# openpifpaf/openpifpaf

Measured on AMD Instinct MI355X. Metric: images/sec end-to-end (backbone+CifCaf decode), resnet50 641px, higher is better.
Workload: dtype f32; 1 GPU; BASELINE configs[1] scaled to a batch: resnet50 641x641, batch 32 per GPU, CIF/CAF fields [32,17,5,81,81]+[32,19,8,81,81]; backbone=resnet50, backbone_dtype=fp32, conv3x3=winograd F(2x2,3x3) f32 for the stride-1 ones, decode_dtype=f32 (+f64 where the reference uses double), global_batch=32, batch_per_gpu=32, parallelism=single GPU, force_complete_pose=False

## Files before the change

openpifpaf_amd/csrc/gemm_f32x3.hip:

```cpp
#include <cstdlib>
#include <type_traits>
#include "common.hpp"
#include "split_bf16.hpp"

namespace opa {

typedef __attribute__((ext_vector_type(8))) __bf16 bf16x8_t;
typedef __attribute__((ext_vector_type(16))) float f32x16_t;
typedef __attribute__((ext_vector_type(4))) float f32x4_t;
typedef __attribute__((ext_vector_type(4))) unsigned int u32x4_t;
typedef __attribute__((ext_vector_type(2))) unsigned int u32x2_t;
typedef __attribute__((ext_vector_type(2))) float f32x2_t;

#ifndef OPA_X3_BK
#define OPA_X3_BK 32
#endif
#ifndef OPA_X3_WGS
#define OPA_X3_WGS 2
#endif
#ifndef OPA_X3_DIAG
#define OPA_X3_DIAG 0
#endif
#ifndef OPA_X3_ONE_ACC
#define OPA_X3_ONE_ACC 0
#endif
#ifndef OPA_X3_SWIZZLE
#define OPA_X3_SWIZZLE 1
#endif
constexpr int kX3BM = 128, kX3BK = OPA_X3_BK, kX3Pitch = OPA_X3_SWIZZLE ? kX3BK : kX3BK + 8;
__device__ __forceinline__ int x3_lds(int row, int k) {
    if (OPA_X3_SWIZZLE && kX3BK == 32) return row * kX3Pitch + ((((k >> 3) ^ (row >> 2)) & 3) << 3) + (k & 7);
    return row * kX3Pitch + k;
}

struct X3Second {
    const float* A2 = nullptr;
    int K1 = 0;
    int ho_wo = 1, wo = 1, hi_wi = 1, wi = 1, stride = 1;
    int hi = 1, C = 0, batch = 1;
    int pix = 1, taps_x = 1, ntaps = 1, padded = 0;
    int dil = 1;
    int lda = 0, ldp = 0, n_real = 0, k_real = 0;
    int act = 0; float act_param = 0.0f;
};

constexpr int kUxAct = 3, kUxHardswish = 2, kUxResidual = 4, kUxActParam = 8;

template <int BN, bool PARTNER, bool RELU, int UX = 0>
__device__ __forceinline__ void x3_unit_epilogue(float* smem_f, const f32x16_t (&acc)[2][BN / 64], const f32x16_t (&low)[2][BN / 64],
                                                 const float* __restrict__ bias, const float* __restrict__ partner,
                                                 float* __restrict__ out, int M, int m0, int n0, int lane, int wave, int ldp, int n_real,
                                                 int act, float act_param) {
    constexpr int WN = BN / 2, NT = WN / 32;
    constexpr int PPR = WN / 2;
    constexpr int PPL = 32 * PPR / 64;
    constexpr int PPRE = PPL > 8 ? 8 : PPL;
    const int wm = wave >> 1, wn = wave & 1;
    float* patch = smem_f + wave * (32 * WN);
#pragma unroll
    for (int i = 0; i < 2; i++) {
        f32x2_t pv[PPRE];
        if (PARTNER) {
#pragma unroll
            for (int t = 0; t < PPRE; t++) {
                const int v = t * 64 + lane;
                const int row = v / PPR, col = n0 + wn * WN + (v % PPR) * 2;
                const int m = m0 + wm * 64 + i * 32 + row;
                pv[t] = (f32x2_t){0.f, 0.f};
                if (m < M && col < n_real) pv[t] = *reinterpret_cast<const f32x2_t*>(partner + (size_t)m * ldp + col);
            }
        }
#pragma unroll
        for (int j = 0; j < NT; j++) {
            const int col = j * 32 + (lane & 31);
            const float b = bias[n0 + wn * WN + col];
#pragma unroll
            for (int r = 0; r < 16; r++) {
                const int row = (r & 3) + 8 * (r >> 2) + 4 * (lane >> 5);
                patch[row * WN + col] = (OPA_X3_ONE_ACC ? acc[i][j][r] : acc[i][j][r] + low[i][j][r]) + b;
            }
        }
        __builtin_amdgcn_fence(__ATOMIC_ACQ_REL, "wavefront");
        __builtin_amdgcn_wave_barrier();
#pragma unroll
        for (int t = 0; t < PPL; t++) {
            const int v = t * 64 + lane;
            const int row = v / PPR, c2 = (v % PPR) * 2, col = n0 + wn * WN + c2;
            const int m = m0 + wm * 64 + i * 32 + row;
            if (m < M && col < n_real) {
                f32x2_t f = *reinterpret_cast<const f32x2_t*>(patch + row * WN + c2);
                if constexpr (PARTNER && (UX & kUxResidual) != 0) {
                    f32x2_t pp;
                    if (t < PPRE) pp = pv[t < PPRE ? t : 0];
                    else pp = *reinterpret_cast<const f32x2_t*>(partner + (size_t)m * ldp + col);
                    f[0] += pp[0]; f[1] += pp[1];
                }
                if (RELU) { f[0] = fmaxf(f[0], 0.0f); f[1] = fmaxf(f[1], 0.0f); }
                if constexpr ((UX & kUxAct) == kUxHardswish) { f[0] = hardswish_f32(f[0]); f[1] = hardswish_f32(f[1]); }
                if constexpr ((UX & kUxActParam) != 0) { f[0] = x3_act_param(f[0], act, act_param); f[1] = x3_act_param(f[1], act, act_param); }
                if (PARTNER && (UX & kUxResidual) == 0) {
                    f32x2_t pp;
                    if (t < PPRE) pp = pv[t < PPRE ? t : 0];
                    else pp = *reinterpret_cast<const f32x2_t*>(partner + (size_t)m * ldp + col);
                    *reinterpret_cast<f32x4_t*>(out + (size_t)m * (2 * (size_t)n_real) + 2 * col) = (f32x4_t){pp[0], f[0], pp[1], f[1]};
                } else {
                    *reinterpret_cast<f32x2_t*>(out + (size_t)m * n_real + col) = f;
                }
            }
        }
        __builtin_amdgcn_fence(__ATOMIC_ACQ_REL, "wavefront");
        __builtin_amdgcn_wave_barrier();
        asm volatile("" ::: "memory");
    }
}

template <int BN, bool RES, bool RELU, bool PRO, int TERMS, int SRC, bool UNIT = false, int UX = 0>
__global__ __launch_bounds__(256, OPA_X3_WGS) void gemm_f32x3_bias_act_kernel(
        const float* __restrict__ A, const unsigned short* __restrict__ W3, const float* __restrict__ bias,
        const float* __restrict__ res, float* __restrict__ out, int M, int N, int K, const float* __restrict__ a_bias,
        const X3Second sec) {
    constexpr int WN = BN / 2;
    constexpr int NT = WN / 32;
    constexpr int LDS_A = kX3BM * kX3Pitch, LDS_B = BN * kX3Pitch;
#ifndef OPA_X3_PAD_LDS
#define OPA_X3_PAD_LDS 0
#endif
    constexpr int STAGE_BYTES = 3 * (LDS_A + LDS_B) * 2 + OPA_X3_PAD_LDS;
    constexpr int EPI_BYTES = 4 * 32 * WN * 4;
    constexpr int SMEM_BYTES = STAGE_BYTES > EPI_BYTES ? STAGE_BYTES : EPI_BYTES;
    __shared__ __attribute__((aligned(16))) unsigned char smem[SMEM_BYTES + (RES && !UNIT ? BN * 4 : 0)];
    unsigned short* sA = reinterpret_cast<unsigned short*>(smem);
    unsigned short* sB = sA + 3 * LDS_A;

    const int tid = threadIdx.x, lane = tid & 63, wave = tid >> 6;
    const int wm = wave >> 1, wn = wave & 1;
    const int n_tiles = N / BN;
    const unsigned nwg = gridDim.x, xcd = blockIdx.x & 7u, in_xcd = blockIdx.x >> 3;
    const unsigned q = nwg >> 3, r8 = nwg & 7u;
    const unsigned logical = (xcd < r8 ? xcd * (q + 1) : r8 * (q + 1) + (xcd - r8) * q) + in_xcd;
    const int m0 = (int)(logical / n_tiles) * kX3BM;
    const int n0 = (int)(logical % n_tiles) * BN;

    constexpr int NL = OPA_X3_ONE_ACC ? 1 : 2;
    f32x16_t acc[2][NT], low_[NL][NT];
    f32x16_t (&low)[2][NT] = OPA_X3_ONE_ACC ? acc : reinterpret_cast<f32x16_t (&)[2][NT]>(low_);
#pragma unroll
    for (int i = 0; i < 2; i++)
#pragma unroll
        for (int j = 0; j < NT; j++)
#pragma unroll
            for (int r = 0; r < 16; r++) { acc[i][j][r] = 0.0f; if (!OPA_X3_ONE_ACC) low[i][j][r] = 0.0f; }

    constexpr int VA = kX3BK / 4;
    constexpr int RPP = 256 / VA;
    constexpr int NPA = kX3BM / RPP;
    constexpr int WQ = kX3BK / 8;
    const int s_row = tid / VA, s_col = (tid % VA) * 4;
    constexpr int WTOT = 3 * BN * WQ;
    constexpr int WV = (WTOT + 255) / 256;
    f32x4_t ra0[NPA], ra1[NPA];
    u32x4_t rb[WV];
    constexpr bool TWO = SRC == 1, TAPS = SRC == 2;
    const int rows_here = M - m0 < kX3BM ? M - m0 : kX3BM;
    const int KA = TWO ? sec.K1 : TAPS ? sec.C : UNIT ? sec.lda : K;
    const int shift = TAPS && !sec.padded ? sec.dil * (sec.wi + 1) * sec.pix : 0;
    const float* a1_base = TAPS ? A - (size_t)shift : A + (size_t)m0 * KA;
    const int a1_bytes = TAPS ? (int)(((size_t)sec.batch * sec.hi_wi * sec.pix + shift) * 4)
                       : UNIT ? (int)(((size_t)(rows_here - 1) * KA + sec.k_real) * 4) : (int)((size_t)rows_here * KA * 4);
    const __amdgpu_buffer_rsrc_t a_rsrc = __builtin_amdgcn_make_buffer_rsrc(const_cast<float*>(a1_base), 0, a1_bytes, 0x00020000);
    const int K2 = K - KA;
    auto in_row = [&](int m) -> long long {
        const int b = m / sec.ho_wo, r = m - b * sec.ho_wo, oy = r / sec.wo, ox = r - oy * sec.wo;
        return (long long)b * sec.hi_wi + (long long)oy * sec.stride * sec.wi + (long long)ox * sec.stride;
    };
    long long row0_2 = 0;
    const float* a2_base = nullptr;
    int a2_bytes = 0;
    unsigned pa2[NPA];
    if constexpr (TWO) {
        row0_2 = in_row(__builtin_amdgcn_readfirstlane(m0));
        const int m_end = m0 + rows_here - 1;
        a2_base = sec.A2 + (size_t)row0_2 * K2;
        a2_bytes = (int)((size_t)(in_row(__builtin_amdgcn_readfirstlane(m_end)) - row0_2 + 1) * K2 * 4);
    }
    const __amdgpu_buffer_rsrc_t w_rsrc = __builtin_amdgcn_make_buffer_rsrc(
        const_cast<unsigned short*>(W3 + (size_t)n0 * K), 0, (int)(((size_t)3 * N - n0) * K * 2), 0x00020000);
    unsigned pa[NPA], pb[WV];
    unsigned vmask[NPA];
    int sb_off[WV];
#pragma unroll
    for (int p = 0; p < NPA; p++) {
        int m = m0 + p * RPP + s_row;
        if (m > M - 1) m = M - 1;
        pa[p] = ((unsigned)(m - m0) * (unsigned)KA + (unsigned)s_col) * 4u;
        vmask[p] = 0u;
        if constexpr (TAPS) {
            const int b = m / sec.ho_wo, r = m - b * sec.ho_wo, oy = r / sec.wo, ox = r - oy * sec.wo;
            pa[p] = (unsigned)((long long)b * sec.hi_wi + (long long)oy * sec.stride * sec.wi + (long long)ox * sec.stride) * (unsigned)sec.pix * 4u
                    + (unsigned)s_col * 4u;
            if (sec.padded) vmask[p] = 0xffffffffu;
            else
                for (int t = 0; t < sec.ntaps; t++) {
                    const int iy = oy * sec.stride - sec.dil + sec.dil * (t / sec.taps_x), ix = ox * sec.stride - sec.dil + sec.dil * (t % sec.taps_x);
                    if (iy >= 0 && iy < sec.hi && ix >= 0 && ix < sec.wi) vmask[p] |= 1u << t;
                }
        }
        if constexpr (TWO) pa2[p] = ((unsigned)(in_row(m) - row0_2) * (unsigned)K2 + (unsigned)s_col) * 4u;
    }
#pragma unroll
    for (int t = 0; t < WV; t++) {
        const int v = t * 256 + tid < WTOT ? t * 256 + tid : WTOT - 1;
        const int plane = v / (BN * WQ), rem = v - plane * (BN * WQ), row = rem / WQ, c = (rem % WQ) * 8;
        pb[t] = (((unsigned)plane * (unsigned)N + (unsigned)row) * (unsigned)K + (unsigned)c) * 2u;
        sb_off[t] = plane * LDS_B + x3_lds(row, c);
    }
    auto fetch_a = [&](f32x4_t (&ra)[NPA], int k0) {
        if constexpr (TAPS) {
            const int t = k0 / KA, kc = k0 - t * KA;
            const int soff = (int)((((unsigned)(sec.dil * (t / sec.taps_x)) * (unsigned)sec.wi + (unsigned)(sec.dil * (t % sec.taps_x))) * (unsigned)sec.pix + (unsigned)kc) * 4u);
#pragma unroll
            for (int p = 0; p < NPA; p++)
                ra[p] = __builtin_bit_cast(f32x4_t, __builtin_amdgcn_raw_buffer_load_b128(a_rsrc, (vmask[p] >> t) & 1u ? pa[p] : 0xFFFFFFF0u, soff, 0));
        } else if constexpr (TWO) {
            const bool second = k0 >= KA;
            const __amdgpu_buffer_rsrc_t rs = __builtin_amdgcn_make_buffer_rsrc(
                const_cast<float*>(second ? a2_base : a1_base), 0, second ? a2_bytes : a1_bytes, 0x00020000);
            const int ks = (second ? k0 - KA : k0) * 4;
#pragma unroll
            for (int p = 0; p < NPA; p++)
                ra[p] = __builtin_bit_cast(f32x4_t, __builtin_amdgcn_raw_buffer_load_b128(rs, second ? pa2[p] : pa[p], ks, 0));
        } else if constexpr (UNIT) {
#pragma unroll
            for (int p = 0; p < NPA; p++) {
                const f32x2_t lo = __builtin_bit_cast(f32x2_t, __builtin_amdgcn_raw_buffer_load_b64(a_rsrc, pa[p], k0 * 4, 0));
                const f32x2_t hi = __builtin_bit_cast(f32x2_t, __builtin_amdgcn_raw_buffer_load_b64(a_rsrc, pa[p] + 8u, k0 * 4, 0));
                ra[p] = (f32x4_t){lo[0], lo[1], hi[0], hi[1]};
            }
        } else {
#pragma unroll
            for (int p = 0; p < NPA; p++) ra[p] = __builtin_bit_cast(f32x4_t, __builtin_amdgcn_raw_buffer_load_b128(a_rsrc, pa[p], k0 * 4, 0));
        }
        if (PRO) {
            const f32x4_t ab = *reinterpret_cast<const f32x4_t*>(a_bias + k0 + s_col);
#pragma unroll
            for (int p = 0; p < NPA; p++)
#pragma unroll
                for (int e = 0; e < 4; e++) ra[p][e] = fmaxf(ra[p][e] + ab[e], 0.0f);
        }
    };
    auto fetch_b = [&](int k0) {
#pragma unroll
        for (int t = 0; t < WV; t++) rb[t] = __builtin_bit_cast(u32x4_t, __builtin_amdgcn_raw_buffer_load_b128(w_rsrc, pb[t], k0 * 2, 0));
    };
    auto store = [&](const f32x4_t (&ra)[NPA], int kt) {
#pragma unroll
        for (int p = 0; p < NPA; p++) {
            u32x2_t p1, p2, p3;
            if (OPA_X3_DIAG == 1) { p1[0] = __float_as_uint(ra[p][0]); p1[1] = __float_as_uint(ra[p][2]); p2 = p1; p3 = p1; }
            else if constexpr (UNIT) {
                const bool in0 = kt + s_col < sec.k_real, in1 = kt + s_col + 2 < sec.k_real;
                const f32x4_t v = {in0 ? ra[p][0] : 0.0f, in0 ? ra[p][1] : 0.0f, in1 ? ra[p][2] : 0.0f, in1 ? ra[p][3] : 0.0f};
                split4(v, p1, p2, p3);
            }
            else split4(ra[p], p1, p2, p3);
            unsigned short* d = sA + x3_lds(p * RPP + s_row, s_col);
            *reinterpret_cast<u32x2_t*>(d) = p1;
            *reinterpret_cast<u32x2_t*>(d + LDS_A) = p2;
            *reinterpret_cast<u32x2_t*>(d + 2 * LDS_A) = p3;
        }
#pragma unroll
        for (int t = 0; t < WV; t++)
            if (WTOT % 256 == 0 || t * 256 + tid < WTOT) *reinterpret_cast<u32x4_t*>(sB + sb_off[t]) = rb[t];
    };
    constexpr int VEC_PER_ROW = WN / 4;
    constexpr int VPL = 32 * VEC_PER_ROW / 64;
    constexpr int VRA = 1;
    constexpr bool TAIL_RES = RES && !UNIT;
    f32x4_t rres[2][TAIL_RES ? VPL : 1];
    auto fetch_res = [&](int i, int t_begin, int t_end) {
        if constexpr (TAIL_RES) {
            const __amdgpu_buffer_rsrc_t r_rsrc = __builtin_amdgcn_make_buffer_rsrc(
                const_cast<float*>(res + (size_t)m0 * N + n0), 0, (int)(((size_t)(rows_here - 1) * N + BN) * 4), 0x00020000);
            const int lrow = wm * 64 + lane / VEC_PER_ROW;
            const unsigned off = ((unsigned)lrow * (unsigned)N + (unsigned)(wn * WN + (lane % VEC_PER_ROW) * 4)) * 4u;
#pragma unroll
            for (int t = t_begin; t < t_end; t++) {
                const int urow = i * 32 + t * (64 / VEC_PER_ROW);
                rres[i][t] = __builtin_bit_cast(f32x4_t, __builtin_amdgcn_raw_buffer_load_b128(
                    r_rsrc, lrow < rows_here - urow ? off : 0xFFFFFFF0u, urow * N * 4, 0));
            }
        }
    };
    int frag_a[kX3BK / 16], frag_b[kX3BK / 16];
    if constexpr (TAIL_RES) {
#pragma unroll
        for (int h = 0; h < kX3BK / 16; h++) {
            frag_a[h] = 2 * x3_lds(wm * 64 + (lane & 31), h * 16 + (lane >> 5) * 8);
            frag_b[h] = 2 * x3_lds(wn * WN + (lane & 31), h * 16 + (lane >> 5) * 8);
            asm volatile("" : "+v"(frag_a[h]), "+v"(frag_b[h]));
        }
    }
    auto step = [&](auto tail, int k0, f32x4_t (&cur)[NPA], f32x4_t (&nxt)[NPA]) {
        constexpr int TAIL = decltype(tail)::value;
        const bool more = TAIL == 1 || (TAIL == 0 && k0 + kX3BK < K);
        const int k_last = K - kX3BK;
        if constexpr (TAIL == 0) {
            fetch_b(k0 + kX3BK < k_last ? k0 + kX3BK : k_last);
            fetch_a(nxt, k0 + 2 * kX3BK < k_last ? k0 + 2 * kX3BK : k_last);
        } else if constexpr (TAIL == 1) {
            fetch_b(k_last);
            fetch_res(0, 0, VRA);
        } else {
            fetch_res(0, VRA, VPL);
        }
        __builtin_amdgcn_sched_barrier(0);
#pragma unroll
        for (int kk = 0; kk < kX3BK; kk += 16) {
            bf16x8_t fa[3][2], fb[3][NT];
            const int kh = OPA_X3_DIAG == 4 ? 0 : kk / 16;
            const int kof = kh * 16 + (lane >> 5) * 8;
#pragma unroll
            for (int pl = 0; pl < 3; pl++) {
#pragma unroll
                for (int i = 0; i < 2; i++)
                    fa[pl][i] = *reinterpret_cast<const bf16x8_t*>(TAIL_RES ? reinterpret_cast<const unsigned short*>(smem + frag_a[kh]) + (pl * LDS_A + i * 32 * kX3Pitch)
                                                                       : sA + pl * LDS_A + x3_lds(wm * 64 + i * 32 + (lane & 31), kof));
#pragma unroll
                for (int j = 0; j < NT; j++)
                    fb[pl][j] = *reinterpret_cast<const bf16x8_t*>(TAIL_RES ? reinterpret_cast<const unsigned short*>(smem + frag_b[kh]) + (3 * LDS_A + pl * LDS_B + j * 32 * kX3Pitch)
                                                                       : sB + pl * LDS_B + x3_lds(wn * WN + j * 32 + (lane & 31), kof));
            }
#pragma unroll
            for (int i = 0; i < 2; i++)
#pragma unroll
                for (int j = 0; j < NT; j++)
                    acc[i][j] = __builtin_amdgcn_mfma_f32_32x32x16_bf16(fa[0][i], fb[0][j], acc[i][j], 0, 0, 0);
#pragma unroll
            for (int s = 4; s >= 1; s--) {
                if ((TERMS == 6 && s > 2) || OPA_X3_DIAG == 3) continue;
#pragma unroll
                for (int pa_ = 0; pa_ < 3; pa_++) {
                    const int pb_ = s - pa_;
                    if (pb_ < 0 || pb_ > 2) continue;
#pragma unroll
                    for (int i = 0; i < 2; i++)
#pragma unroll
                        for (int j = 0; j < NT; j++)
                            low[i][j] = __builtin_amdgcn_mfma_f32_32x32x16_bf16(fa[pa_][i], fb[pb_][j], low[i][j], 0, 0, 0);
                }
            }
        }
        __syncthreads();
        if (more && (OPA_X3_DIAG != 2 || cur[0][0] == 12345.678f)) store(cur, k0 + kX3BK);
        __syncthreads();
    };
    fetch_b(0);
    fetch_a(ra0, 0);
    if constexpr (TAIL_RES) {
        if (tid < BN) reinterpret_cast<float*>(smem + SMEM_BYTES)[tid] = bias[n0 + tid];
    }
    store(ra0, 0);
    __syncthreads();
    fetch_a(ra1, kX3BK);
    constexpr std::integral_constant<int, 0> any_step{};
    if constexpr (TAIL_RES) {
        int k0 = 0;
        for (; k0 < K - 2 * kX3BK; k0 += 2 * kX3BK) {
            step(any_step, k0, ra1, ra0);
            step(any_step, k0 + kX3BK, ra0, ra1);
        }
        step(std::integral_constant<int, 1>{}, k0, ra1, ra0);
        step(std::integral_constant<int, 2>{}, k0 + kX3BK, ra0, ra1);
    } else {
        for (int k0 = 0; k0 < K; k0 += 2 * kX3BK) {
            step(any_step, k0, ra1, ra0);
            step(any_step, k0 + kX3BK, ra0, ra1);
        }
    }
    if constexpr (UNIT) {
        x3_unit_epilogue<BN, RES, RELU, UX>(reinterpret_cast<float*>(smem), acc, low, bias, res, out, M, m0, n0, lane, wave, sec.ldp, sec.n_real,
                                            sec.act, sec.act_param);
        return;
    }

    float* patch = reinterpret_cast<float*>(smem) + wave * (32 * WN);
    if constexpr (TAIL_RES) {
        fetch_res(1, 0, VPL);
        __builtin_amdgcn_sched_barrier(0);
    }
#pragma unroll
    for (int i = 0; i < 2; i++) {
#pragma unroll
        for (int j = 0; j < NT; j++) {
            const int col = j * 32 + (lane & 31);
            const float b = TAIL_RES ? reinterpret_cast<const float*>(smem + SMEM_BYTES)[wn * WN + col] : bias[n0 + wn * WN + col];
#pragma unroll
            for (int r = 0; r < 16; r++) {
                const int row = (r & 3) + 8 * (r >> 2) + 4 * (lane >> 5);
                patch[row * WN + col] = (OPA_X3_ONE_ACC ? acc[i][j][r] : acc[i][j][r] + low[i][j][r]) + b;
            }
        }
        __builtin_amdgcn_fence(__ATOMIC_ACQ_REL, "wavefront");
        __builtin_amdgcn_wave_barrier();
#pragma unroll
        for (int t = 0; t < VPL; t++) {
            const int v = t * 64 + lane;
            const int row = v / VEC_PER_ROW, c4 = (v % VEC_PER_ROW) * 4;
            const int m = m0 + wm * 64 + i * 32 + row;
            if (m < M) {
                f32x4_t f = *reinterpret_cast<const f32x4_t*>(patch + row * WN + c4);
                if constexpr (TAIL_RES) f += rres[i][t];
                if (RELU) {
#pragma unroll
                    for (int e = 0; e < 4; e++) f[e] = fmaxf(f[e], 0.0f);
                }
                *reinterpret_cast<f32x4_t*>(out + (size_t)m * N + n0 + wn * WN + c4) = f;
            }
        }
        __builtin_amdgcn_fence(__ATOMIC_ACQ_REL, "wavefront");
        __builtin_amdgcn_wave_barrier();
        asm volatile("" ::: "memory");
    }
}

#if OPA_X3_BK == 32 && OPA_X3_SWIZZLE && !OPA_X3_ONE_ACC && OPA_X3_DIAG == 0
#define OPA_X3_HAS_WIDE 1
constexpr int kX3WideBN = 256, kX3WideThreads = 512;
constexpr int kX3WideStageBytes = 3 * (kX3BM + kX3WideBN) * kX3Pitch * 2;
constexpr int kX3WideLdsBytes = 2 * kX3WideStageBytes + kX3WideBN * 4;
constexpr unsigned kX3WideCUs = 256;
constexpr int kX3WideMinKRes = 768;
constexpr bool x3_wide_pays(unsigned long long wide_blocks, bool res, int K) {
    if (res && K < kX3WideMinKRes) return false;
    const unsigned long long rounds = (wide_blocks + kX3WideCUs - 1) / kX3WideCUs;
    return wide_blocks >= 2 * kX3WideCUs && rounds * kX3WideCUs * 15 <= (wide_blocks + kX3WideCUs / 4) * 16;
}

template <bool RES, bool RELU, bool PRO, int SRC>
__global__ __launch_bounds__(kX3WideThreads, 2) void gemm_f32x3_wide_kernel(
        const float* __restrict__ A, const unsigned short* __restrict__ W3, const float* __restrict__ bias,
        const float* __restrict__ res, float* __restrict__ out, int M, int N, int K, const float* __restrict__ a_bias,
        const X3Second sec) {
    constexpr int BN = kX3WideBN, WN = 64, NT = 2;
    constexpr int LDS_A = kX3BM * kX3Pitch, LDS_B = BN * kX3Pitch;
    static_assert(kX3WideThreads / 64 * 32 * WN * 4 <= kX3WideStageBytes, "the epilogue patches alias stage 0 alone");
    extern __shared__ __attribute__((aligned(16))) unsigned char x3w_smem[];
    float* s_bias = reinterpret_cast<float*>(x3w_smem + 2 * kX3WideStageBytes);

    const int tid = threadIdx.x, lane = tid & 63, wave = __builtin_amdgcn_readfirstlane(tid >> 6);
    const int wm = wave >> 2, wn = wave & 3;
    const int n_tiles = N / BN;
    const unsigned nwg = gridDim.x, xcd = blockIdx.x & 7u, in_xcd = blockIdx.x >> 3;
    const unsigned q = nwg >> 3, r8 = nwg & 7u;
    const unsigned logical = (xcd < r8 ? xcd * (q + 1) : r8 * (q + 1) + (xcd - r8) * q) + in_xcd;
    const int m0 = (int)(logical / n_tiles) * kX3BM;
    const int n0 = (int)(logical % n_tiles) * BN;

    f32x16_t acc[2][NT], low[2][NT];
#pragma unroll
    for (int i = 0; i < 2; i++)
#pragma unroll
        for (int j = 0; j < NT; j++)
#pragma unroll
            for (int r = 0; r < 16; r++) { acc[i][j][r] = 0.0f; low[i][j][r] = 0.0f; }

    constexpr int VA = kX3BK / 4, RPP = kX3WideThreads / VA, NPA = kX3BM / RPP, WV = 6;
    static_assert(NPA == 2 && 3 * BN * (kX3BK / 8) == WV * kX3WideThreads, "staging maps");
    const int s_row = tid / VA, s_col = (tid % VA) * 4;
    f32x4_t ra0[NPA], ra1[NPA], ab0, ab1;
    u32x4_t rb[WV];
    constexpr bool TWO = SRC == 1, TAPS = SRC == 2;
    const int rows_here = M - m0 < kX3BM ? M - m0 : kX3BM;
    const int KA = TWO ? sec.K1 : TAPS ? sec.C : K;
    const int shift = TAPS && !sec.padded ? sec.dil * (sec.wi + 1) * sec.pix : 0;
    const float* a1_base = TAPS ? A - (size_t)shift : A + (size_t)m0 * KA;
    const int a1_bytes = TAPS ? (int)(((size_t)sec.batch * sec.hi_wi * sec.pix + shift) * 4) : (int)((size_t)rows_here * KA * 4);
    const __amdgpu_buffer_rsrc_t a_rsrc = __builtin_amdgcn_make_buffer_rsrc(const_cast<float*>(a1_base), 0, a1_bytes, 0x00020000);
    const int K2 = K - KA;
    auto in_row = [&](int m) -> long long {
        const int b = m / sec.ho_wo, r = m - b * sec.ho_wo, oy = r / sec.wo, ox = r - oy * sec.wo;
        return (long long)b * sec.hi_wi + (long long)oy * sec.stride * sec.wi + (long long)ox * sec.stride;
    };
    long long row0_2 = 0;
    const float* a2_base = nullptr;
    int a2_bytes = 0;
    unsigned pa2[NPA];
    if constexpr (TWO) {
        row0_2 = in_row(__builtin_amdgcn_readfirstlane(m0));
        const int m_end = m0 + rows_here - 1;
        a2_base = sec.A2 + (size_t)row0_2 * K2;
        a2_bytes = (int)((size_t)(in_row(__builtin_amdgcn_readfirstlane(m_end)) - row0_2 + 1) * K2 * 4);
    }
    const __amdgpu_buffer_rsrc_t w_rsrc = __builtin_amdgcn_make_buffer_rsrc(
        const_cast<unsigned short*>(W3 + (size_t)n0 * K), 0, (int)(((size_t)3 * N - n0) * K * 2), 0x00020000);
    unsigned pa[NPA], vmask[NPA];
#pragma unroll
    for (int p = 0; p < NPA; p++) {
        int m = m0 + p * RPP + s_row;
        if (m > M - 1) m = M - 1;
        pa[p] = ((unsigned)(m - m0) * (unsigned)KA + (unsigned)s_col) * 4u;
        vmask[p] = 0u;
        if constexpr (TAPS) {
            const int b = m / sec.ho_wo, r = m - b * sec.ho_wo, oy = r / sec.wo, ox = r - oy * sec.wo;
            pa[p] = (unsigned)((long long)b * sec.hi_wi + (long long)oy * sec.stride * sec.wi + (long long)ox * sec.stride) * (unsigned)sec.pix * 4u
                    + (unsigned)s_col * 4u;
            if (sec.padded) vmask[p] = 0xffffffffu;
            else
                for (int t = 0; t < sec.ntaps; t++) {
                    const int iy = oy * sec.stride - sec.dil + sec.dil * (t / sec.taps_x), ix = ox * sec.stride - sec.dil + sec.dil * (t % sec.taps_x);
                    if (iy >= 0 && iy < sec.hi && ix >= 0 && ix < sec.wi) vmask[p] |= 1u << t;
                }
        }
        if constexpr (TWO) pa2[p] = ((unsigned)(in_row(m) - row0_2) * (unsigned)K2 + (unsigned)s_col) * 4u;
    }
    const unsigned pb = ((unsigned)(tid >> 2) * (unsigned)K + (unsigned)(tid & 3) * 8u) * 2u;
    const int sb_off = x3_lds(tid >> 2, (tid & 3) * 8);
    const int sa_off = x3_lds(s_row, s_col);
    auto fetch_a = [&](f32x4_t (&ra)[NPA], f32x4_t& ab, int k0) {
        if constexpr (TAPS) {
            const int t = k0 / KA, kc = k0 - t * KA;
            const int soff = (int)((((unsigned)(sec.dil * (t / sec.taps_x)) * (unsigned)sec.wi + (unsigned)(sec.dil * (t % sec.taps_x))) * (unsigned)sec.pix + (unsigned)kc) * 4u);
#pragma unroll
            for (int p = 0; p < NPA; p++)
                ra[p] = __builtin_bit_cast(f32x4_t, __builtin_amdgcn_raw_buffer_load_b128(a_rsrc, (vmask[p] >> t) & 1u ? pa[p] : 0xFFFFFFF0u, soff, 0));
        } else if constexpr (TWO) {
            const bool second = k0 >= KA;
            const __amdgpu_buffer_rsrc_t rs = __builtin_amdgcn_make_buffer_rsrc(
                const_cast<float*>(second ? a2_base : a1_base), 0, second ? a2_bytes : a1_bytes, 0x00020000);
            const int ks = (second ? k0 - KA : k0) * 4;
#pragma unroll
            for (int p = 0; p < NPA; p++)
                ra[p] = __builtin_bit_cast(f32x4_t, __builtin_amdgcn_raw_buffer_load_b128(rs, second ? pa2[p] : pa[p], ks, 0));
        } else {
#pragma unroll
            for (int p = 0; p < NPA; p++) ra[p] = __builtin_bit_cast(f32x4_t, __builtin_amdgcn_raw_buffer_load_b128(a_rsrc, pa[p], k0 * 4, 0));
        }
        if (PRO) ab = *reinterpret_cast<const f32x4_t*>(a_bias + k0 + s_col);
    };
    auto fetch_b = [&](int k0) {
#pragma unroll
        for (int t = 0; t < WV; t++)
            rb[t] = __builtin_bit_cast(u32x4_t, __builtin_amdgcn_raw_buffer_load_b128(
                w_rsrc, pb, (int)((((unsigned)(t >> 1) * (unsigned)N + (unsigned)(t & 1) * 128u) * (unsigned)K + (unsigned)k0) * 2u), 0));
    };
    auto store_a = [&](const f32x4_t (&ra)[NPA], const f32x4_t& ab, int stage) {
        unsigned short* sA = reinterpret_cast<unsigned short*>(x3w_smem + stage * kX3WideStageBytes);
#pragma unroll
        for (int p = 0; p < NPA; p++) {
            f32x4_t v = ra[p];
            if (PRO) {
#pragma unroll
                for (int e = 0; e < 4; e++) v[e] = fmaxf(v[e] + ab[e], 0.0f);
            }
            u32x2_t p1, p2, p3;
            split4(v, p1, p2, p3);
            unsigned short* d = sA + sa_off + p * RPP * kX3Pitch;
            *reinterpret_cast<u32x2_t*>(d) = p1;
            *reinterpret_cast<u32x2_t*>(d + LDS_A) = p2;
            *reinterpret_cast<u32x2_t*>(d + 2 * LDS_A) = p3;
        }
    };
    auto store_b = [&](int stage) {
        unsigned short* sB = reinterpret_cast<unsigned short*>(x3w_smem + stage * kX3WideStageBytes) + 3 * LDS_A;
#pragma unroll
        for (int t = 0; t < WV; t++)
            *reinterpret_cast<u32x4_t*>(sB + (t >> 1) * LDS_B + (t & 1) * 128 * kX3Pitch + sb_off) = rb[t];
    };
    constexpr int VEC_PER_ROW = WN / 4, VPL = 32 * VEC_PER_ROW / 64, VRA = 1;
    f32x4_t rres[2][RES ? VPL : 1];
    auto fetch_res = [&](int i, int t_begin, int t_end) {
        if constexpr (RES) {
            const __amdgpu_buffer_rsrc_t r_rsrc = __builtin_amdgcn_make_buffer_rsrc(
                const_cast<float*>(res + (size_t)m0 * N + n0), 0, (int)(((size_t)(rows_here - 1) * N + BN) * 4), 0x00020000);
            const int lrow = wm * 64 + lane / VEC_PER_ROW;
            const unsigned off = ((unsigned)lrow * (unsigned)N + (unsigned)(wn * WN + (lane % VEC_PER_ROW) * 4)) * 4u;
#pragma unroll
            for (int t = t_begin; t < t_end; t++) {
                const int urow = i * 32 + t * (64 / VEC_PER_ROW);
                rres[i][t] = __builtin_bit_cast(f32x4_t, __builtin_amdgcn_raw_buffer_load_b128(
                    r_rsrc, lrow < rows_here - urow ? off : 0xFFFFFFF0u, urow * N * 4, 0));
            }
        }
    };
    int frag_a[2], frag_b[2];
#pragma unroll
    for (int h = 0; h < 2; h++) {
        frag_a[h] = 2 * x3_lds(wm * 64 + (lane & 31), h * 16 + (lane >> 5) * 8);
        frag_b[h] = 2 * (3 * LDS_A + x3_lds(wn * WN + (lane & 31), h * 16 + (lane >> 5) * 8));
        asm volatile("" : "+v"(frag_a[h]), "+v"(frag_b[h]));
    }
    auto multiply = [&](int stage) {
        const unsigned char* base = x3w_smem + stage * kX3WideStageBytes;
#pragma unroll
        for (int kh = 0; kh < 2; kh++) {
            bf16x8_t fa[3][2], fb[3][NT];
#pragma unroll
            for (int pl = 0; pl < 3; pl++) {
#pragma unroll
                for (int i = 0; i < 2; i++)
                    fa[pl][i] = *reinterpret_cast<const bf16x8_t*>(reinterpret_cast<const unsigned short*>(base + frag_a[kh]) + (pl * LDS_A + i * 32 * kX3Pitch));
#pragma unroll
                for (int j = 0; j < NT; j++)
                    fb[pl][j] = *reinterpret_cast<const bf16x8_t*>(reinterpret_cast<const unsigned short*>(base + frag_b[kh]) + (pl * LDS_B + j * 32 * kX3Pitch));
            }
#pragma unroll
            for (int i = 0; i < 2; i++)
#pragma unroll
                for (int j = 0; j < NT; j++)
                    acc[i][j] = __builtin_amdgcn_mfma_f32_32x32x16_bf16(fa[0][i], fb[0][j], acc[i][j], 0, 0, 0);
#pragma unroll
            for (int s = 2; s >= 1; s--) {
#pragma unroll
                for (int pa_ = 0; pa_ < 3; pa_++) {
                    const int pb_ = s - pa_;
                    if (pb_ < 0 || pb_ > 2) continue;
#pragma unroll
                    for (int i = 0; i < 2; i++)
#pragma unroll
                        for (int j = 0; j < NT; j++)
                            low[i][j] = __builtin_amdgcn_mfma_f32_32x32x16_bf16(fa[pa_][i], fb[pb_][j], low[i][j], 0, 0, 0);
                }
            }
        }
    };
    auto step = [&](auto tail, auto stage_c, int k0, f32x4_t (&cur)[NPA], f32x4_t& cur_ab, f32x4_t (&nxt)[NPA], f32x4_t& nxt_ab) {
        constexpr int TAIL = decltype(tail)::value, STAGE = decltype(stage_c)::value;
        if constexpr (TAIL == 0) {
            fetch_b(k0 + kX3BK);
            fetch_a(nxt, nxt_ab, k0 + 2 * kX3BK);
        } else if constexpr (TAIL == 1) {
            fetch_b(k0 + kX3BK);
            fetch_res(0, 0, VRA);
        } else {
            fetch_res(0, VRA, VPL);
        }
        __builtin_amdgcn_sched_barrier(0);
        multiply(STAGE);
        if constexpr (TAIL != 2) {
            store_a(cur, cur_ab, STAGE ^ 1);
#pragma unroll
            for (int g = 0; g < 44; g++) {
                __builtin_amdgcn_sched_group_barrier(0x008, 1, 0);
                __builtin_amdgcn_sched_group_barrier(0x002, 1, 0);
            }
            store_b(STAGE ^ 1);
        }
        __syncthreads();
    };
    const float bias_v = bias[n0 + (tid & (BN - 1))];
    fetch_b(0);
    fetch_a(ra0, ab0, 0);
    fetch_a(ra1, ab1, kX3BK);
    if (tid < BN) s_bias[tid] = bias_v;
    store_a(ra0, ab0, 0);
    store_b(0);
    __syncthreads();
    constexpr std::integral_constant<int, 0> c0{};
    constexpr std::integral_constant<int, 1> c1{};
    constexpr std::integral_constant<int, 2> c2{};
    int k0 = 0;
    for (; k0 < K - 2 * kX3BK; k0 += 2 * kX3BK) {
        step(c0, c0, k0, ra1, ab1, ra0, ab0);
        step(c0, c1, k0 + kX3BK, ra0, ab0, ra1, ab1);
    }
    step(c1, c0, k0, ra1, ab1, ra0, ab0);
    step(c2, c1, k0 + kX3BK, ra0, ab0, ra1, ab1);

    float* patch = reinterpret_cast<float*>(x3w_smem) + wave * (32 * WN);
    if constexpr (RES) {
        fetch_res(1, 0, VPL);
        __builtin_amdgcn_sched_barrier(0);
    }
#pragma unroll
    for (int i = 0; i < 2; i++) {
#pragma unroll
        for (int j = 0; j < NT; j++) {
            const int col = j * 32 + (lane & 31);
            const float b = s_bias[wn * WN + col];
#pragma unroll
            for (int r = 0; r < 16; r++) {
                const int row = (r & 3) + 8 * (r >> 2) + 4 * (lane >> 5);
                patch[row * WN + col] = acc[i][j][r] + low[i][j][r] + b;
            }
        }
        __builtin_amdgcn_fence(__ATOMIC_ACQ_REL, "wavefront");
        __builtin_amdgcn_wave_barrier();
#pragma unroll
        for (int t = 0; t < VPL; t++) {
            const int v = t * 64 + lane;
            const int row = v / VEC_PER_ROW, c4 = (v % VEC_PER_ROW) * 4;
            const int m = m0 + wm * 64 + i * 32 + row;
            if (m < M) {
                f32x4_t f = *reinterpret_cast<const f32x4_t*>(patch + row * WN + c4);
                if constexpr (RES) f += rres[i][t];
                if (RELU) {
#pragma unroll
                    for (int e = 0; e < 4; e++) f[e] = fmaxf(f[e], 0.0f);
                }
                *reinterpret_cast<f32x4_t*>(out + (size_t)m * N + n0 + wn * WN + c4) = f;
            }
        }
        __builtin_amdgcn_fence(__ATOMIC_ACQ_REL, "wavefront");
        __builtin_amdgcn_wave_barrier();
        asm volatile("" ::: "memory");
    }
}
#else
#define OPA_X3_HAS_WIDE 0
#endif

enum X3Mode { kX3Plain = 0, kX3Pair = 1, kX3Taps = 2, kX3Unit = 3 };

constexpr bool x3_exists(int BN, bool RES, bool RELU, bool PRO, int TERMS, int SRC, bool UNIT, int UX) {
    if (!UNIT) return UX == 0 && !(SRC != 0 && RES) && !(SRC == 2 && PRO);
    if (SRC != 0 || PRO || (BN == 128 && TERMS == 9)) return false;
    const bool known = UX == 0 || UX == kUxHardswish || UX == kUxResidual || UX == (kUxResidual | kUxHardswish) || UX == kUxActParam;
    return known && !(RELU && (UX & ~kUxResidual) != 0) && !((UX & kUxResidual) != 0 && !RES);
}

static hipError_t launch_x3(X3Mode mode, const float* A, const unsigned short* W3, const float* bias, const float* third, float* out,
                            int M, int N, int K, bool relu, int ux, int terms, const float* a_bias, hipStream_t st, const X3Second& sec) {
    const int bn = mode != kX3Unit ? (N % 128 == 0 ? 128 : 64)
                                   : (N % 128 == 0 && terms == 6 ? 128 : 64);
    const unsigned blocks = (unsigned)((long long)((M + kX3BM - 1) / kX3BM) * (N / bn));
#if OPA_X3_HAS_WIDE
    if (mode != kX3Unit && terms == 6 && N % kX3WideBN == 0) {
        const char* env = std::getenv("OPA_X3_TILE");
        const int forced = env && *env ? std::atoi(env) : 0;
        const unsigned wide_blocks = blocks / 2;
        if (forced == kX3WideBN || (forced != 128 && x3_wide_pays(wide_blocks, third != nullptr, K)))
            return with_value<kX3Plain, kX3Pair, kX3Taps>(mode, [&](auto MODE) {
            return with_flag(third != nullptr, [&](auto RES) {
            return with_flag(relu, [&](auto RELU) {
            return with_flag(a_bias != nullptr, [&](auto PRO) {
                constexpr int SRC = (int)decltype(MODE)::value;
                if constexpr (x3_exists(kX3WideBN, RES, RELU, PRO, 6, SRC, false, 0)) {
                    auto* kernel = &gemm_f32x3_wide_kernel<RES, RELU, PRO, SRC>;
                    hipError_t e = hipFuncSetAttribute(reinterpret_cast<const void*>(kernel), hipFuncAttributeMaxDynamicSharedMemorySize, kX3WideLdsBytes);
                    if (e != hipSuccess) return e;
                    kernel<<<wide_blocks, kX3WideThreads, kX3WideLdsBytes, st>>>(A, W3, bias, third, out, M, N, K, a_bias, sec);
                    return hipGetLastError();
                } else {
                    return hipErrorInvalidValue;
                }
            }); }); }); });
    }
#endif
    return with_value<64, 128>(bn, [&](auto BN) {
    return with_value<6, 9>(terms == 6 ? 6 : 9, [&](auto TERMS) {
    return with_value<kX3Plain, kX3Pair, kX3Taps, kX3Unit>(mode, [&](auto MODE) {
    return with_value<0, kUxHardswish, kUxResidual, kUxResidual | kUxHardswish, kUxActParam>(ux, [&](auto UX) {
    return with_flag(third != nullptr, [&](auto RES) {
    return with_flag(relu, [&](auto RELU) {
    return with_flag(a_bias != nullptr, [&](auto PRO) {
        constexpr bool UNIT = MODE == kX3Unit;
        constexpr int SRC = UNIT ? 0 : (int)MODE;
        if constexpr (x3_exists(BN, RES, RELU, PRO, TERMS, SRC, UNIT, UX)) {
            gemm_f32x3_bias_act_kernel<BN, RES, RELU, PRO, TERMS, SRC, UNIT, UX><<<blocks, 256, 0, st>>>(A, W3, bias, third, out, M, N, K, a_bias, sec);
            return hipGetLastError();
        } else {
            return hipErrorInvalidValue;
        }
    }); }); }); }); }); }); });
}

hipError_t launch_gemm_f32x3_bias_act(const float* A, const unsigned short* W3, const float* bias, const float* res, float* out,
                                      int M, int N, int K, int relu, int terms, hipStream_t st, const float* a_bias) {
    return launch_x3(kX3Plain, A, W3, bias, res, out, M, N, K, relu != 0, 0, terms, a_bias, st, X3Second{});
}

hipError_t launch_gemm2_f32x3_bias_act(const float* A1, int K1, const float* A2, int K2, int batch, int hi, int wi, int stride,
                                       const unsigned short* W3, const float* bias, float* out, int N, int relu, int terms,
                                       hipStream_t st, const float* a_bias) {
    const int ho = (hi - 1) / stride + 1, wo = (wi - 1) / stride + 1;
    X3Second sec;
    sec.A2 = A2; sec.K1 = K1;
    sec.ho_wo = ho * wo; sec.wo = wo; sec.hi_wi = hi * wi; sec.wi = wi; sec.stride = stride;
    return launch_x3(kX3Pair, A1, W3, bias, nullptr, out, batch * ho * wo, N, K1 + K2, relu != 0, 0, terms, a_bias, st, sec);
}

hipError_t launch_gemm_unit_act_f32x3(const float* A, int lda, const unsigned short* W3, const float* bias, const float* partner, int ldp,
                                      const float* residual, int ldr, float* out, int M, int N, int K, int act, int terms, hipStream_t st,
                                      float act_param) {
    if ((partner && residual) || act < 0 || act > 4) return hipErrorInvalidValue;
    X3Second sec;
    sec.lda = lda; sec.ldp = residual ? ldr : ldp; sec.n_real = N; sec.k_real = K;
    if (act >= 3) { sec.act = act; sec.act_param = act_param; }
    const int ux = (act == 2 ? kUxHardswish : 0) | (act >= 3 ? kUxActParam : 0) | (residual ? kUxResidual : 0);
    const int Np = (N + 63) / 64 * 64, Kp = (K + 63) / 64 * 64;
    return launch_x3(kX3Unit, A, W3, bias, residual ? residual : partner, out, M, Np, Kp, act == 1, ux, terms, nullptr, st, sec);
}

hipError_t launch_conv3x3_f32x3(const float* x, int batch, int hi, int wi, int C, int stride, int dilation, const unsigned short* W3,
                                const float* bias, float* out, int N, int relu, int terms, hipStream_t st) {
    const int ho = (hi - 1) / stride + 1, wo = (wi - 1) / stride + 1;
    X3Second sec;
    sec.ho_wo = ho * wo; sec.wo = wo; sec.hi_wi = hi * wi; sec.wi = wi; sec.stride = stride;
    sec.hi = hi; sec.C = C; sec.batch = batch;
    sec.pix = C; sec.taps_x = 3; sec.ntaps = 9; sec.dil = dilation;
    return launch_x3(kX3Taps, x, W3, bias, nullptr, out, batch * ho * wo, N, 9 * C, relu != 0, 0, terms, nullptr, st, sec);
}

hipError_t launch_convrows_f32x3(const float* x, int batch, int hp, int wp, int pix, int ho, int wo, int stride, int ntaps, int tap_floats,
                                 const unsigned short* W3, const float* bias, float* out, int N, int relu, int terms, hipStream_t st) {
    X3Second sec;
    sec.ho_wo = ho * wo; sec.wo = wo; sec.hi_wi = hp * wp; sec.wi = wp; sec.stride = stride;
    sec.hi = hp; sec.C = tap_floats; sec.batch = batch;
    sec.pix = pix; sec.taps_x = 1; sec.ntaps = ntaps; sec.padded = 1;
    return launch_x3(kX3Taps, x, W3, bias, nullptr, out, batch * ho * wo, N, ntaps * tap_floats, relu != 0, 0, terms, nullptr, st, sec);
}

}
```

Measured before the change: 682.3 images/s.

## Split wide GEMM tail-wave tiles into half-height blocks to balance the last round

```diff
diff --git a/openpifpaf_amd/csrc/gemm_f32x3.hip b/openpifpaf_amd/csrc/gemm_f32x3.hip
--- a/openpifpaf_amd/csrc/gemm_f32x3.hip
+++ b/openpifpaf_amd/csrc/gemm_f32x3.hip
@@ -430,18 +430,99 @@
 constexpr int kX3WideLdsBytes = 2 * kX3WideStageBytes + kX3WideBN * 4;
 constexpr unsigned kX3WideCUs = 256;
 constexpr int kX3WideMinKRes = 768;
+constexpr unsigned kX3WideRemMaxRounds = 8;
+constexpr bool x3_wide_rem_pays(unsigned long long wide_blocks) {
+    const unsigned long long r = wide_blocks % kX3WideCUs;
+    return wide_blocks >= 2 * kX3WideCUs && wide_blocks <= kX3WideRemMaxRounds * kX3WideCUs && r != 0 && 2 * r <= kX3WideCUs;
+}
 constexpr bool x3_wide_pays(unsigned long long wide_blocks, bool res, int K) {
     if (res && K < kX3WideMinKRes) return false;
-    const unsigned long long rounds = (wide_blocks + kX3WideCUs - 1) / kX3WideCUs;
-    return wide_blocks >= 2 * kX3WideCUs && rounds * kX3WideCUs * 15 <= (wide_blocks + kX3WideCUs / 4) * 16;
-}
-
-template <bool RES, bool RELU, bool PRO, int SRC>
-__global__ __launch_bounds__(kX3WideThreads, 2) void gemm_f32x3_wide_kernel(
+    const unsigned long long r = wide_blocks % kX3WideCUs;
+    const unsigned long long tenths = wide_blocks / kX3WideCUs * 10 + (r == 0 ? 0 : x3_wide_rem_pays(wide_blocks) ? 5 : 10);
+    return wide_blocks >= 2 * kX3WideCUs && tenths * kX3WideCUs * 15 <= (wide_blocks + kX3WideCUs / 4) * 16 * 10;
+}
+constexpr unsigned x3_wide_grid(unsigned wide_blocks, bool halves) {
+    return halves ? wide_blocks + wide_blocks % kX3WideCUs : wide_blocks;
+}
+
+struct X3WideTile { int m0, rows, n0; };
+constexpr unsigned x3_xcd_order(unsigned i, unsigned n) {
+    const unsigned xcd = i & 7u, in_xcd = i >> 3, q = n >> 3, r8 = n & 7u;
+    return (xcd < r8 ? xcd * (q + 1) : r8 * (q + 1) + (xcd - r8) * q) + in_xcd;
+}
+constexpr X3WideTile x3_wide_map(unsigned block, unsigned grid, unsigned full, unsigned n_tiles) {
+    if (block < full) {
+        const unsigned t = x3_xcd_order(block, full);
+        return {(int)(t / n_tiles) * kX3BM, kX3BM, (int)(t % n_tiles) * kX3WideBN};
+    }
+    const unsigned h = x3_xcd_order(block - full, grid - full), t = full + h / 2;
+    return {(int)(t / n_tiles) * kX3BM + (int)(h & 1u) * (kX3BM / 2), kX3BM / 2, (int)(t % n_tiles) * kX3WideBN};
+}
+constexpr bool x3_xcd_order_permutes(unsigned n) {
+    unsigned long long sum = 0, sq = 0;
+    for (unsigned i = 0; i < n; i++) {
+        const unsigned long long l = x3_xcd_order(i, n);
+        if (l >= n) return false;
+        sum += l; sq += l * l;
+    }
+    const unsigned long long f = n;
+    return f == 0 || (sum == f * (f - 1) / 2 && sq == (f - 1) * f * (2 * f - 1) / 6);
+}
+constexpr bool x3_wide_map_covers(unsigned row_tiles, unsigned n_tiles, bool halves) {
+    const unsigned tiles = row_tiles * n_tiles, grid = x3_wide_grid(tiles, halves);
+    const unsigned full = halves ? tiles / kX3WideCUs * kX3WideCUs : tiles;
+    if (grid - full != 2 * (tiles - full)) return false;
+    for (unsigned b = 0; b < full; b = b + 61 < full || b == full - 1 ? b + 61 : full - 1) {
+        const X3WideTile t = x3_wide_map(b, grid, full, n_tiles);
+        if (t.rows != kX3BM || t.m0 % kX3BM != 0 || t.n0 % kX3WideBN != 0) return false;
+        if ((unsigned)(t.m0 / kX3BM) * n_tiles + t.n0 / kX3WideBN != x3_xcd_order(b, full) || t.n0 / kX3WideBN >= (int)n_tiles) return false;
+    }
+    bool seen[2 * kX3WideCUs] = {};
+    for (unsigned b = full; b < grid; b++) {
+        const X3WideTile t = x3_wide_map(b, grid, full, n_tiles);
+        if (t.rows != kX3BM / 2 || t.m0 % (kX3BM / 2) != 0 || t.n0 % kX3WideBN != 0 || t.n0 / kX3WideBN >= (int)n_tiles) return false;
+        const unsigned tile = (unsigned)(t.m0 / kX3BM) * n_tiles + t.n0 / kX3WideBN;
+        if (tile < full || tile >= tiles) return false;
+        const unsigned s = (tile - full) * 2 + t.m0 % kX3BM / (kX3BM / 2);
+        if (seen[s]) return false;
+        seen[s] = true;
+    }
+    return true;
+}
+constexpr bool x3_wide_map_ok(unsigned row_tiles, unsigned n_tiles) {
+    const unsigned tiles = row_tiles * n_tiles, full = tiles / kX3WideCUs * kX3WideCUs;
+    return x3_wide_map_covers(row_tiles, n_tiles, false) && x3_wide_map_covers(row_tiles, n_tiles, true) &&
+           x3_xcd_order_permutes(2 * (tiles - full));
+}
+static_assert(x3_wide_map_ok(1641, 1) && x3_wide_map_ok(842, 1) && x3_wide_map_ok(842, 2) && x3_wide_map_ok(3282, 1) &&
+              x3_wide_map_ok(1641, 2) && x3_wide_map_ok(6481, 1) && x3_wide_map_ok(25761, 1), "the step's launches");
+static_assert(x3_xcd_order_permutes(1641) && x3_xcd_order_permutes(1536) && x3_xcd_order_permutes(842) && x3_xcd_order_permutes(768), "");
+static_assert(x3_xcd_order_permutes(3282) && x3_xcd_order_permutes(3072) && x3_xcd_order_permutes(6481) && x3_xcd_order_permutes(6400), "");
+static_assert(x3_xcd_order_permutes(25761), "");
+static_assert(x3_xcd_order_permutes(25600), "");
+static_assert(x3_wide_map_ok(512, 1) && x3_wide_map_ok(513, 1) && x3_wide_map_ok(640, 1) && x3_wide_map_ok(641, 1) &&
+              x3_wide_map_ok(1, 1) && x3_wide_map_ok(100, 1) && x3_wide_map_ok(129, 2) && x3_wide_map_ok(171, 3) &&
+              x3_wide_map_ok(421, 8), "edge cases");
+static_assert(x3_wide_grid(1641, true) == 1536 + 210 && x3_wide_grid(842, true) == 768 + 148 && x3_wide_grid(512, true) == 512 &&
+              x3_wide_grid(1641, false) == 1641, "grid sizes");
+static_assert(x3_wide_map(0, 258, 256, 2).rows == 128 && x3_wide_map(256, 258, 256, 2).m0 == 128 * kX3BM &&
+              x3_wide_map(256, 258, 256, 2).n0 == 0 && x3_wide_map(257, 258, 256, 2).m0 == 128 * kX3BM + 64 &&
+              x3_wide_map(257, 258, 256, 2).rows == 64, "129 row tiles x 2 column tiles: one tile left over, as two halves");
+static_assert(x3_wide_rem_pays(1641) && x3_wide_rem_pays(842) && !x3_wide_rem_pays(6481) && !x3_wide_rem_pays(3282) &&
+              !x3_wide_rem_pays(3368) && !x3_wide_rem_pays(25761) && !x3_wide_rem_pays(512) && x3_wide_rem_pays(513) &&
+              x3_wide_rem_pays(640) && !x3_wide_rem_pays(641) && !x3_wide_rem_pays(200), "where the remainder runs half-height");
+static_assert(x3_wide_pays(1641, false, 1024) && x3_wide_pays(842, false, 2048) && x3_wide_pays(3282, false, 1024) &&
+              x3_wide_pays(6481, false, 512) && x3_wide_pays(25761, false, 128) && x3_wide_pays(3368, false, 1536) &&
+              !x3_wide_pays(500, false, 1024) && !x3_wide_pays(3368, true, 512), "the step's launches under the rule");
+static_assert(x3_wide_pays(600, false, 1024) && x3_wide_pays(1030, false, 1024) && x3_wide_pays(1300, false, 1024) &&
+              !x3_wide_pays(641, false, 1024) && !x3_wide_pays(650, false, 1024), "the sweep's points under the rule");
+
+template <int MB, bool RES, bool RELU, bool PRO, int SRC>
+__device__ __forceinline__ void x3_wide_tile(
         const float* __restrict__ A, const unsigned short* __restrict__ W3, const float* __restrict__ bias,
         const float* __restrict__ res, float* __restrict__ out, int M, int N, int K, const float* __restrict__ a_bias,
-        const X3Second sec) {
-    constexpr int BN = kX3WideBN, WN = 64, NT = 2;
+        const X3Second& sec, const int m0, const int n0) {
+    constexpr int BN = kX3WideBN, WN = 64, NT = 2, BM = MB * 64;
     constexpr int LDS_A = kX3BM * kX3Pitch, LDS_B = BN * kX3Pitch;
     static_assert(kX3WideThreads / 64 * 32 * WN * 4 <= kX3WideStageBytes, "the epilogue patches alias stage 0 alone");
     extern __shared__ __attribute__((aligned(16))) unsigned char x3w_smem[];
@@ -449,28 +530,22 @@
 
     const int tid = threadIdx.x, lane = tid & 63, wave = __builtin_amdgcn_readfirstlane(tid >> 6);
     const int wm = wave >> 2, wn = wave & 3;
-    const int n_tiles = N / BN;
-    const unsigned nwg = gridDim.x, xcd = blockIdx.x & 7u, in_xcd = blockIdx.x >> 3;
-    const unsigned q = nwg >> 3, r8 = nwg & 7u;
-    const unsigned logical = (xcd < r8 ? xcd * (q + 1) : r8 * (q + 1) + (xcd - r8) * q) + in_xcd;
-    const int m0 = (int)(logical / n_tiles) * kX3BM;
-    const int n0 = (int)(logical % n_tiles) * BN;
-
-    f32x16_t acc[2][NT], low[2][NT];
-#pragma unroll
-    for (int i = 0; i < 2; i++)
+
+    f32x16_t acc[MB][NT], low[MB][NT];
+#pragma unroll
+    for (int i = 0; i < MB; i++)
 #pragma unroll
         for (int j = 0; j < NT; j++)
 #pragma unroll
             for (int r = 0; r < 16; r++) { acc[i][j][r] = 0.0f; low[i][j][r] = 0.0f; }
 
-    constexpr int VA = kX3BK / 4, RPP = kX3WideThreads / VA, NPA = kX3BM / RPP, WV = 6;
-    static_assert(NPA == 2 && 3 * BN * (kX3BK / 8) == WV * kX3WideThreads, "staging maps");
+    constexpr int VA = kX3BK / 4, RPP = kX3WideThreads / VA, NPA = BM / RPP, WV = 6;
+    static_assert(NPA == MB && 3 * BN * (kX3BK / 8) == WV * kX3WideThreads, "staging maps");
     const int s_row = tid / VA, s_col = (tid % VA) * 4;
     f32x4_t ra0[NPA], ra1[NPA], ab0, ab1;
     u32x4_t rb[WV];
     constexpr bool TWO = SRC == 1, TAPS = SRC == 2;
-    const int rows_here = M - m0 < kX3BM ? M - m0 : kX3BM;
+    const int rows_here = M - m0 < BM ? M - m0 : BM;
     const int KA = TWO ? sec.K1 : TAPS ? sec.C : K;
     const int shift = TAPS && !sec.padded ? sec.dil * (sec.wi + 1) * sec.pix : 0;
     const float* a1_base = TAPS ? A - (size_t)shift : A + (size_t)m0 * KA;
@@ -567,12 +642,12 @@
             *reinterpret_cast<u32x4_t*>(sB + (t >> 1) * LDS_B + (t & 1) * 128 * kX3Pitch + sb_off) = rb[t];
     };
     constexpr int VEC_PER_ROW = WN / 4, VPL = 32 * VEC_PER_ROW / 64, VRA = 1;
-    f32x4_t rres[2][RES ? VPL : 1];
+    f32x4_t rres[MB][RES ? VPL : 1];
     auto fetch_res = [&](int i, int t_begin, int t_end) {
         if constexpr (RES) {
             const __amdgpu_buffer_rsrc_t r_rsrc = __builtin_amdgcn_make_buffer_rsrc(
                 const_cast<float*>(res + (size_t)m0 * N + n0), 0, (int)(((size_t)(rows_here - 1) * N + BN) * 4), 0x00020000);
-            const int lrow = wm * 64 + lane / VEC_PER_ROW;
+            const int lrow = wm * (BM / 2) + lane / VEC_PER_ROW;
             const unsigned off = ((unsigned)lrow * (unsigned)N + (unsigned)(wn * WN + (lane % VEC_PER_ROW) * 4)) * 4u;
 #pragma unroll
             for (int t = t_begin; t < t_end; t++) {
@@ -585,7 +660,7 @@
     int frag_a[2], frag_b[2];
 #pragma unroll
     for (int h = 0; h < 2; h++) {
-        frag_a[h] = 2 * x3_lds(wm * 64 + (lane & 31), h * 16 + (lane >> 5) * 8);
+        frag_a[h] = 2 * x3_lds(wm * (BM / 2) + (lane & 31), h * 16 + (lane >> 5) * 8);
         frag_b[h] = 2 * (3 * LDS_A + x3_lds(wn * WN + (lane & 31), h * 16 + (lane >> 5) * 8));
         asm volatile("" : "+v"(frag_a[h]), "+v"(frag_b[h]));
     }
@@ -593,18 +668,18 @@
         const unsigned char* base = x3w_smem + stage * kX3WideStageBytes;
 #pragma unroll
         for (int kh = 0; kh < 2; kh++) {
-            bf16x8_t fa[3][2], fb[3][NT];
+            bf16x8_t fa[3][MB], fb[3][NT];
 #pragma unroll
             for (int pl = 0; pl < 3; pl++) {
 #pragma unroll
-                for (int i = 0; i < 2; i++)
+                for (int i = 0; i < MB; i++)
                     fa[pl][i] = *reinterpret_cast<const bf16x8_t*>(reinterpret_cast<const unsigned short*>(base + frag_a[kh]) + (pl * LDS_A + i * 32 * kX3Pitch));
 #pragma unroll
                 for (int j = 0; j < NT; j++)
                     fb[pl][j] = *reinterpret_cast<const bf16x8_t*>(reinterpret_cast<const unsigned short*>(base + frag_b[kh]) + (pl * LDS_B + j * 32 * kX3Pitch));
             }
 #pragma unroll
-            for (int i = 0; i < 2; i++)
+            for (int i = 0; i < MB; i++)
 #pragma unroll
                 for (int j = 0; j < NT; j++)
                     acc[i][j] = __builtin_amdgcn_mfma_f32_32x32x16_bf16(fa[0][i], fb[0][j], acc[i][j], 0, 0, 0);
@@ -615,7 +690,7 @@
                     const int pb_ = s - pa_;
                     if (pb_ < 0 || pb_ > 2) continue;
 #pragma unroll
-                    for (int i = 0; i < 2; i++)
+                    for (int i = 0; i < MB; i++)
 #pragma unroll
                         for (int j = 0; j < NT; j++)
                             low[i][j] = __builtin_amdgcn_mfma_f32_32x32x16_bf16(fa[pa_][i], fb[pb_][j], low[i][j], 0, 0, 0);
@@ -639,7 +714,7 @@
         if constexpr (TAIL != 2) {
             store_a(cur, cur_ab, STAGE ^ 1);
 #pragma unroll
-            for (int g = 0; g < 44; g++) {
+            for (int g = 0; g < 22 * MB; g++) {
                 __builtin_amdgcn_sched_group_barrier(0x008, 1, 0);
                 __builtin_amdgcn_sched_group_barrier(0x002, 1, 0);
             }
@@ -667,12 +742,12 @@
     step(c2, c1, k0 + kX3BK, ra0, ab0, ra1, ab1);
 
     float* patch = reinterpret_cast<float*>(x3w_smem) + wave * (32 * WN);
-    if constexpr (RES) {
+    if constexpr (RES && MB == 2) {
         fetch_res(1, 0, VPL);
         __builtin_amdgcn_sched_barrier(0);
     }
 #pragma unroll
-    for (int i = 0; i < 2; i++) {
+    for (int i = 0; i < MB; i++) {
 #pragma unroll
         for (int j = 0; j < NT; j++) {
             const int col = j * 32 + (lane & 31);
@@ -689,7 +764,7 @@
         for (int t = 0; t < VPL; t++) {
             const int v = t * 64 + lane;
             const int row = v / VEC_PER_ROW, c4 = (v % VEC_PER_ROW) * 4;
-            const int m = m0 + wm * 64 + i * 32 + row;
+            const int m = m0 + wm * (BM / 2) + i * 32 + row;
             if (m < M) {
                 f32x4_t f = *reinterpret_cast<const f32x4_t*>(patch + row * WN + c4);
                 if constexpr (RES) f += rres[i][t];
@@ -703,6 +778,23 @@
         __builtin_amdgcn_fence(__ATOMIC_ACQ_REL, "wavefront");
         __builtin_amdgcn_wave_barrier();
         asm volatile("" ::: "memory");
+    }
+}
+
+template <bool RES, bool RELU, bool PRO, int SRC, bool REM>
+__global__ __launch_bounds__(kX3WideThreads, 2) void gemm_f32x3_wide_kernel(
+        const float* __restrict__ A, const unsigned short* __restrict__ W3, const float* __restrict__ bias,
+        const float* __restrict__ res, float* __restrict__ out, int M, int N, int K, const float* __restrict__ a_bias,
+        const X3Second sec) {
+    const unsigned n_tiles = (unsigned)(N / kX3WideBN);
+    if constexpr (REM) {
+        const unsigned tiles = (unsigned)((M + kX3BM - 1) / kX3BM) * n_tiles;
+        const X3WideTile t = x3_wide_map(blockIdx.x, gridDim.x, tiles / kX3WideCUs * kX3WideCUs, n_tiles);
+        if (t.rows == kX3BM) x3_wide_tile<2, RES, RELU, PRO, SRC>(A, W3, bias, res, out, M, N, K, a_bias, sec, t.m0, t.n0);
+        else if (t.m0 < M) x3_wide_tile<1, RES, RELU, PRO, SRC>(A, W3, bias, res, out, M, N, K, a_bias, sec, t.m0, t.n0);
+    } else {
+        const X3WideTile t = x3_wide_map(blockIdx.x, gridDim.x, gridDim.x, n_tiles);
+        x3_wide_tile<2, RES, RELU, PRO, SRC>(A, W3, bias, res, out, M, N, K, a_bias, sec, t.m0, t.n0);
     }
 }
 #else
@@ -728,22 +820,27 @@
         const char* env = std::getenv("OPA_X3_TILE");
         const int forced = env && *env ? std::atoi(env) : 0;
         const unsigned wide_blocks = blocks / 2;
-        if (forced == kX3WideBN || (forced != 128 && x3_wide_pays(wide_blocks, third != nullptr, K)))
+        if (forced == kX3WideBN || (forced != 128 && x3_wide_pays(wide_blocks, third != nullptr, K))) {
+            const char* rem_env = std::getenv("OPA_X3_REM");
+            const bool halves = wide_blocks % kX3WideCUs != 0 &&
+                                (rem_env && *rem_env ? std::atoi(rem_env) != 0 : x3_wide_rem_pays(wide_blocks));
+            return with_flag(halves, [&](auto REM) {
             return with_value<kX3Plain, kX3Pair, kX3Taps>(mode, [&](auto MODE) {
             return with_flag(third != nullptr, [&](auto RES) {
             return with_flag(relu, [&](auto RELU) {
             return with_flag(a_bias != nullptr, [&](auto PRO) {
                 constexpr int SRC = (int)decltype(MODE)::value;
                 if constexpr (x3_exists(kX3WideBN, RES, RELU, PRO, 6, SRC, false, 0)) {
-                    auto* kernel = &gemm_f32x3_wide_kernel<RES, RELU, PRO, SRC>;
+                    auto* kernel = &gemm_f32x3_wide_kernel<RES, RELU, PRO, SRC, REM>;
                     hipError_t e = hipFuncSetAttribute(reinterpret_cast<const void*>(kernel), hipFuncAttributeMaxDynamicSharedMemorySize, kX3WideLdsBytes);
                     if (e != hipSuccess) return e;
-                    kernel<<<wide_blocks, kX3WideThreads, kX3WideLdsBytes, st>>>(A, W3, bias, third, out, M, N, K, a_bias, sec);
+                    kernel<<<x3_wide_grid(wide_blocks, REM), kX3WideThreads, kX3WideLdsBytes, st>>>(A, W3, bias, third, out, M, N, K, a_bias, sec);
                     return hipGetLastError();
                 } else {
                     return hipErrorInvalidValue;
                 }
-            }); }); }); });
+            }); }); }); }); });
+        }
     }
 #endif
     return with_value<64, 128>(bn, [&](auto BN) {
```

Measured after the change: 685.0 images/s, median of 6. About the same (+0.4%).
